# wbuntine/libstb

Measured on AMD Instinct MI355X. Metric: S-table cells/s, higher is better.
Workload: dtype f64

## Files before the change

include/stb_hip.h:

```cpp
#ifndef STB_HIP_H
#define STB_HIP_H

#include <stddef.h>
#include <stdint.h>

#ifdef __cplusplus
extern "C" {
#endif

const char *stb_last_error(void);
int stb_device_count(void);
int stb_device_name(char *buf, int len);

int stb_set_device(int dev);
int stb_get_device(void);
int stb_device_enter(int dev);
void stb_device_leave(int prev);

void *stb_device_malloc(size_t bytes);
void stb_device_free(void *p);
void *stb_host_malloc(size_t bytes);
void stb_host_free(void *p);
void *stb_host_malloc_huge(size_t bytes);
void stb_host_free_huge(void *p);
// ... 170 lines not shown
int stb_groups_aterms_multi(stb_groups_t *const *sets, int k, const double *x_host, int D, double *out_host);
int stb_groups_create_node(int ndev, int I, const int *K, const uint32_t *T, const uint32_t *nflat, const uint16_t *tflat,
                           const double *bpar, unsigned N, unsigned M, int Dmax, stb_groups_t **sets_out);
int stb_groups_aterms_device(stb_groups_t *g, const double *x_host, int D, double *d_out, void *stream);
int stb_groups_ssum_device(stb_groups_t *g, const double *x_host, int D, double *d_out, void *stream);
int stb_groups_ssum(stb_groups_t *g, const double *x_host, int D, double *out_host);
int stb_groups_aterms_tables(stb_groups_t *g, const double *x_host, int D, double *out_host);
double stb_groups_samplea(stb_groups_t *g, double a, void *rng, int loops, int verbose);
typedef struct stb_modea_info {
  int rounds, evals, at_bound;
  double lo, hi, g_lo, g_hi;
  double grad, delta;
} stb_modea_info_t;
int stb_groups_aterms_grad(stb_groups_t *g, const double *x_host, int D, double *val_out, double *grad_out);
int stb_groups_modea(stb_groups_t *g, double a_lo, double a_hi, double tol, int rounds_max, double *a_hat, double *curv,
                     stb_modea_info_t *info);
int stb_groups_update_restaurants(stb_groups_t *g, const uint32_t *T, const double *bpar);
int stb_groups_pairs_begin(stb_groups_t *g);
int stb_groups_pairs_put(stb_groups_t *g, const uint32_t *n, const uint16_t *t, uint64_t count, unsigned *maxn, unsigned *maxt);
int stb_groups_pairs_put_ragged(stb_groups_t *g, int I, const int *K, uint32_t *const *n, uint16_t *const *t, unsigned *maxn, unsigned *maxt);
int stb_groups_pairs_commit(stb_groups_t *g, const uint32_t *T, const double *bpar, unsigned N, unsigned M);
int stb_groups_update_pairs(stb_groups_t *g, const uint32_t *nflat, const uint16_t *tflat);
unsigned stb_groups_fallbacks(void);
int stb_grid_shape(unsigned N, unsigned M, int D, int *C_out, int *G_out, int *K_out);
int stb_groups_shape(const stb_groups_t *g, int *I, uint64_t *G, unsigned *N, unsigned *M, int *Dmax);
int stb_groups_last_form(const stb_groups_t *g, int *fused, int *which, int *sparse, int *C, int *R);
int stb_groups_aterms_timed(stb_groups_t *g, const double *x_host, int D, double *out_host,
                            float *ms_fill, float *ms_sweep, float *ms_terms);

int stb_sample_tcounts(const double *d_table, const double *d_S1, unsigned N, unsigned M, double a,
                       const double *d_bpar, int I, const uint64_t *d_koff , const uint32_t *d_n,
                       uint16_t *d_t, uint32_t *d_T, const double *d_h ,
                       uint64_t seed, uint64_t sweep, void *stream);
typedef struct stb_tcounts stb_tcounts_t;
stb_tcounts_t *stb_tcounts_create(int I, const int *K, const uint32_t *nflat, const uint16_t *tflat,
                                  const double *hflat, unsigned M );
int stb_tcounts_set_h(stb_tcounts_t *s, const double *hflat);
int stb_tcounts_sweep(stb_tcounts_t *s, double a, const double *bpar ,
                      uint64_t seed, uint64_t sweep, int nsweeps);
int stb_tcounts_get(stb_tcounts_t *s, uint16_t *t_out, uint32_t *T_out);
int stb_tcounts_to_groups(stb_tcounts_t *s, stb_groups_t *g, const double *bpar );
double stb_tcounts_sampleb(stb_tcounts_t *s, double b_in, double shape, double scale, double a, void *rng,
                           int loops, int verbose, uint64_t seed, uint64_t sweep);
void stb_tcounts_free(stb_tcounts_t *s);

#define STB_TC_REF_WINDOW 1u
// ... 213 lines not shown
```

libstb_amd/capi.py:

```python
from __future__ import annotations

import ctypes as C
import os
from functools import lru_cache

import numpy as np

_HERE = os.path.dirname(os.path.abspath(__file__))
LIB_PATH = os.environ.get("STB_LIB_PATH") or os.path.join(_HERE, "lib", "libstb_amd.so")

S_STABLE, S_UVTABLE, S_FLOAT, S_VERBOSE, S_QUITONBOUND, S_THREADS, S_ASYMPT = 1, 2, 4, 8, 16, 32, 64
FILL_SCALED, FILL_LOGDOMAIN, FILL_SCALED_STEP, FILL_SPLIT, FILL_FUSED, FILL_PC, FILL_CHAIN, FILL_CHAINX, FILL_CK, FILL_HB = 0, 1, 2, 3, 4, 5, 6, 7, 8, 9

c_double_p = C.POINTER(C.c_double)
c_u32_p = C.POINTER(C.c_uint32)
c_u16_p = C.POINTER(C.c_uint16)
c_int_p = C.POINTER(C.c_int)
c_float_p = C.POINTER(C.c_float)

LOGDENS = C.CFUNCTYPE(C.c_double, C.c_double, C.c_void_p)
GETVAL = C.CFUNCTYPE(None, c_u32_p, c_u16_p, C.c_uint, C.c_uint)


class StbError(RuntimeError):
# ... 98 lines not shown
    _fields_ = [("stages", C.c_int), ("accepted", C.c_int), ("evals", C.c_int), ("stage_pick", C.c_int),
                ("log_alpha", C.c_double), ("rect", C.c_double * 4), ("a_prop", C.c_double), ("b_prop", C.c_double),
                ("L_cur", C.c_double), ("L_prop", C.c_double), ("cell", C.c_int * 5), ("box", (C.c_int * 4) * 5),
                ("L", c_double_p)]


@lru_cache(maxsize=None)
def lib() -> C.CDLL:
    if not os.path.exists(LIB_PATH):
        raise StbError(
            f"{LIB_PATH} is missing: build it with `python -c 'import __graft_entry__ as g; g.build()'` "
            "or `make -C libstb_amd/csrc` (there is no pure-Python or CPU implementation)")
    try:
        import torch
    except Exception:
        pass
    L = C.CDLL(LIB_PATH)
    u, d, i, vp, u64, sz = C.c_uint, C.c_double, C.c_int, C.c_void_p, C.c_uint64, C.c_size_t

    ROUND5 = {"stb_groups_pairs_begin", "stb_groups_pairs_put", "stb_groups_pairs_put_ragged", "stb_groups_pairs_commit",
              "stb_groups_update_pairs", "stb_groups_fallbacks", "stb_grid_shape", "stb_bterms_update",
              "stb_table_probe", "stb_slow_launches", "stb_shared_gpu_mode", "stb_set_shared_gpu", "stb_note_launch_span",
              "stb_lookup_V", "stb_lookup_U", "stb_lookup_UV", "stb_groups_aterms_multi", "stb_groups_create_node",
              "stb_groups_last_form"}

    def sig(name, res, args):
        try:
            f = getattr(L, name)
        except AttributeError:
            if name in ROUND5 and os.environ.get("STB_LIB_PATH"):
                return
            raise
        f.restype = res
        f.argtypes = args

    sig("S_make", vp, [u, u, u, u, d, C.c_uint32])
    sig("S_tag", None, [vp, C.c_char_p])
    sig("S_remake", i, [vp, d])
    sig("S_free", None, [vp])
    for n in ("S_S", "S_U", "S_UV", "S_V", "S_asympt"):
        sig(n, d, [vp, u, u])
    sig("S_S1", d, [vp, u])
    sig("S_report", None, [vp, vp])
    sig("stb_extend_policy", None, [u, u, u, u, i, i, C.POINTER(u), C.POINTER(u)])
    sig("stb_table_sync", i, [vp])
    sig("stb_table_probe", None, [vp, i, C.POINTER(u), C.POINTER(u), sz, c_double_p])
    sig("stb_table_mirrored", None, [vp, C.POINTER(u), C.POINTER(u)])
# ... 46 lines not shown
    sig("stb_lookup_U", i, [vp, u, u, C.c_double, vp, vp, u64, vp, vp])
    sig("stb_lookup_UV", i, [vp, u, u, C.c_double, vp, vp, u64, vp, vp])
    sig("stb_sweep_workspace_bytes", sz, [u64, i])
    sig("stb_sweep_S", i, [vp, u64, vp, u64, i, u, u, vp, vp, u64, vp, vp, sz, vp])
    sig("stb_terms_workspace_bytes", sz, [u64, i])
    sig("stb_restaurant_terms", i, [c_double_p, i, vp, vp, u64, vp, vp, sz, vp])
    sig("stb_bterms", i, [c_double_p, i, d, d, d, vp, u64, vp, vp, sz, vp])
    sig("stb_groups_create", vp, [i, c_int_p, c_u32_p, c_u32_p, c_u16_p, c_double_p, u, u, i])
    sig("stb_groups_free", None, [vp])
    sig("stb_groups_aterms", i, [vp, c_double_p, i, c_double_p])
    sig("stb_groups_aterms_tables", i, [vp, c_double_p, i, c_double_p])
    sig("stb_groups_aterms_async", i, [vp, c_double_p, i, c_double_p, vp])
    sig("stb_groups_wait", i, [vp])
    sig("stb_groups_aterms_multi", i, [C.POINTER(vp), i, c_double_p, i, c_double_p])
    sig("stb_groups_create_node", i, [i, i, c_int_p, c_u32_p, c_u32_p, c_u16_p, c_double_p, u, u, i, C.POINTER(vp)])
    sig("stb_groups_aterms_device", i, [vp, c_double_p, i, vp, vp])
    sig("stb_groups_update_restaurants", i, [vp, c_u32_p, c_double_p])
    sig("stb_groups_pairs_begin", i, [vp])
    sig("stb_groups_pairs_put", i, [vp, c_u32_p, c_u16_p, u64, C.POINTER(u), C.POINTER(u)])
    sig("stb_groups_pairs_put_ragged", i, [vp, i, c_int_p, vp, vp, C.POINTER(u), C.POINTER(u)])
    sig("stb_groups_pairs_commit", i, [vp, c_u32_p, c_double_p, u, u])
    sig("stb_groups_update_pairs", i, [vp, c_u32_p, c_u16_p])
    sig("stb_groups_fallbacks", C.c_uint, [])
    sig("stb_grid_shape", i, [u, u, i, c_int_p, c_int_p, c_int_p])
    sig("stb_groups_shape", i, [vp, c_int_p, C.POINTER(u64), C.POINTER(u), C.POINTER(u), c_int_p])
    sig("stb_groups_last_form", i, [vp, c_int_p, c_int_p, c_int_p, c_int_p, c_int_p])
    sig("stb_sampler_cache_clear", None, [])
    sig("stb_groups_aterms_timed", i, [vp, c_double_p, i, c_double_p, c_float_p, c_float_p, c_float_p])
    sig("stb_sample_tcounts", i, [vp, vp, u, u, d, vp, i, vp, vp, vp, vp, vp, u64, u64, vp])
    sig("stb_tcounts_create", vp, [i, c_int_p, c_u32_p, c_u16_p, c_double_p, u])
    sig("stb_tcounts_set_h", i, [vp, c_double_p])
    sig("stb_tcounts_sweep", i, [vp, d, c_double_p, u64, u64, i])
    sig("stb_tcounts_get", i, [vp, c_u16_p, c_u32_p])
    sig("stb_tcounts_to_groups", i, [vp, vp, c_double_p])
    sig("stb_tcounts_free", None, [vp])
    sig("stb_sample_tcounts_window", i, [vp, vp, u, u, d, vp, i, vp, vp, vp, vp, vp, u, u, u64, u64, vp])
    sig("stb_tcounts_sweep_window", i, [vp, d, c_double_p, u, u, u64, u64, i])
    sig("stb_sample_tindic", i, [vp, u, u, d, vp, i, vp, vp, vp, vp, vp, vp, vp, u, u64, u64, vp])
    sig("stb_tindic_create", vp, [i, c_int_p, c_u32_p, c_u16_p, c_double_p, c_u32_p, u, u])
    sig("stb_tindic_set_h", i, [vp, c_double_p])
    sig("stb_tindic_sweep", i, [vp, d, c_double_p, u64, u64, i])
    sig("stb_tindic_get", i, [vp, c_u16_p, c_u32_p])
    sig("stb_tindic_to_groups", i, [vp, vp, c_double_p])
    sig("stb_tindic_free", None, [vp])
    sig("stb_sample_tdishes", i, [vp, u, u, d, vp, i, vp, vp, vp, vp, vp, vp, vp, vp, vp, u, u, u64, u64, vp, vp])
    sig("stb_tindic_set_classes", i, [vp, c_u32_p, u])
# ... 1189 lines not shown
```

libstb_amd/csrc/groups.h:

```cpp
#ifndef STB_GROUPS_H
#define STB_GROUPS_H

#include <vector>

#include "stb_common.h"

#define STB_TERMS_DMAX 64
#define STB_NLISTS 6
#define GH_JQ_HOST 64
#define STB_WS_FORM 4096

struct slab_info {
  int R, G, NQ, UC, HC;
  int PB;
  unsigned UCp;
  const unsigned *rec_off;
};

struct stb_cell_list {
  unsigned *item_ptr;
  unsigned short *ent_pos;
  unsigned *ent_cnt;
  unsigned *tile_off, *dense, *tinfo, *jobs, *tjob, *tnw, *toff;
  unsigned n_jobs;
  int ready, R, G;
  size_t ent_cap, dense_cap;
};
static inline bool stb_list_from_slab(const stb_cell_list &l) { return l.ent_cap != 0; }


struct stb_groups {
  int dev;
  int I;
  uint64_t G;
  unsigned N, M;
  int Dmax;
  uint32_t *d_n, *d_T;
  uint16_t *d_t;
  double *d_bpar;
  double *d_tables, *d_S1, *d_out;
// ... 28 lines not shown
  int pend_ssum;
  int sel_which;
  int last_fused, last_C, last_R;
  double *pend_out;
  double pend_x[STB_TERMS_DMAX];
  last_fill pend_fill;
  uint32_t *h_pn;
  uint16_t *h_pt;
  uint32_t *h_T;
  double *h_bpar;
  uint64_t put_n, flushed_n;
  unsigned put_maxn, put_maxt;
  int putting;
  int have_pairs;
  int have_bounds;
  int sorted;
  unsigned *d_slab;
  size_t slab_elems;
  int slab_which;
  int slab_R, slab_G, slab_UCp;
  unsigned slab_items;
  int slab_clean;
  unsigned *d_icnt;
  unsigned long long *d_ninf;
  void *d_scan_tmp;
  size_t scan_tmp_bytes;
  double *d_gtab, *d_dS1g, *d_gout;
  void *d_ws_da, *d_ws_dasweep;
  size_t ws_da, ws_dasweep;
  uint64_t da_stride, da_G;
  unsigned da_N, da_M;
};

static inline int stb_grid_which(int C) { return C == 2 ? 3 : (C == 4 ? 4 : 5); }
static inline int stb_which_C(int which) { return which == 3 ? 2 : (which == 4 ? 4 : 8); }
static inline int stb_pos_bits(int C) { return C == 8 ? 9 : 8; }

#if defined(__HIPCC__)
__device__ __forceinline__ unsigned stb_block_exclusive_1024(unsigned mine, unsigned *lds, unsigned *total) {
  const unsigned tid = threadIdx.x, lane = tid & 63, wave = tid >> 6;
  unsigned v = mine;
#pragma unroll
  for (int o = 1; o < 64; o <<= 1) {
    const unsigned u = __shfl_up(v, o, 64);
    if ((int)lane >= o) v += u;
  }
  if (lane == 63) lds[wave] = v;
  __syncthreads();
  if (tid == 0) {
// ... 7 lines not shown
  }
  __syncthreads();
  const unsigned ex = lds[wave] + v - mine;
  if (total) *total = lds[16];
  __syncthreads();
  return ex;
}
#endif

#define STB_DENSE_NWMAX 40
#define STB_DENSE_CSR 63u

void stb_grid_tile_offsets(const grid_geom &g, std::vector<unsigned> &off);

void stb_list_release(stb_cell_list &l, bool with_shape);
void stb_lists_drop(stb_groups_t *g, bool keep_capacity);
void stb_list_request(const stb_groups_t *g, int which, dot_request *req);
int stb_lists_build(stb_groups_t *g, int which, int D);
int stb_lists_slab_build(stb_groups_t *g, int which, int D, const hb_dot_info &H, const grid_geom &gg);
int stb_lists_jobs_device(stb_groups_t *g, int which, int D, const grid_geom &gg, const unsigned *tnw);
int stb_lists_jobs_from(stb_groups_t *g, int which, int D, const grid_geom &gg, const unsigned *h_nw);
int stb_lists_sort_build(stb_groups_t *g, int which, int D, const hb_dot_info &H, const grid_geom &gg);
void stb_groups_new_pairs(stb_groups_t *g, int reused);
int stb_groups_set_bounds(stb_groups_t *g, unsigned N, unsigned M);
int stb_groups_sort_pairs(stb_groups_t *g);
int stb_groups_alloc_dotp(stb_groups_t *g);

struct stb_counts_view {
  int dev, I;
  uint64_t G;
  unsigned maxn, Mdraw;
  const uint32_t *d_n, *d_T;
  const uint16_t *d_t;
  const double *d_bpar;
  bool resident;
  hipStream_t st;
  const char *noun;
};
int stb_groups_take_counts(stb_groups_t *g, const stb_counts_view &v, const double *bpar, const char *who);

#endif
```

libstb_amd/csrc/groups.hip:

```cpp

#include <rocprim/device/device_radix_sort.hpp>

#include <atomic>

#include "groups.h"

__global__ void k_pack_pairs(const uint32_t *n, const uint16_t *t, uint64_t G, uint64_t *key) {
  uint64_t g = (uint64_t)blockIdx.x * blockDim.x + threadIdx.x;
  if (g < G) key[g] = ((uint64_t)n[g] << 16) | t[g];
}
__global__ void k_unpack_pairs(const uint64_t *key, uint64_t G, uint32_t *n, uint16_t *t) {
  uint64_t g = (uint64_t)blockIdx.x * blockDim.x + threadIdx.x;
  if (g < G) {
    n[g] = (uint32_t)(key[g] >> 16);
    t[g] = (uint16_t)(key[g] & 0xffff);
  }
}

static int sort_pairs(uint32_t *d_n, uint16_t *d_t, uint64_t G, hipStream_t st) {
  if (G < 2) return 0;
  uint64_t *k0 = nullptr, *k1 = nullptr;
  void *tmp = nullptr;
  size_t tmp_bytes = 0;
  int rc = 1;
// ... 15 lines not shown
    if (rocprim::radix_sort_keys(tmp, tmp_bytes, k0, k1, (size_t)G, 0, 48, st) != hipSuccess) {
      stb_fail("sort_pairs: radix_sort_keys failed");
      break;
    }
    hipLaunchKernelGGL(k_unpack_pairs, dim3(blocks), dim3(256), 0, st, k1, G, d_n, d_t);
    if (hipStreamSynchronize(st) != hipSuccess) {
      stb_fail("sort_pairs: %s", hipGetErrorString(hipGetLastError()));
      break;
    }
    rc = 0;
  } while (0);
  if (rc != 0) (void)hipStreamSynchronize(st);
  stb_pool_free(k0);
  stb_pool_free(k1);
  stb_pool_free(tmp);
  return rc;
}

extern "C" void stb_groups_free(stb_groups_t *g) {
  STB_ENTRY;
  if (!g) return;
  stb_device_scope dev(g->dev);
  std::vector<void *> ptrs = {g->d_n, g->d_T, g->d_t, g->d_bpar, g->d_tables, g->d_S1, g->d_out, g->d_ws_fill, g->d_ws_sweep, g->d_ws_terms,
                              g->d_cnt, g->d_n2, g->d_t2, g->d_dotp, g->d_slab, g->d_icnt, g->d_ninf, g->d_scan_tmp,
                              g->d_gtab, g->d_dS1g, g->d_gout, g->d_ws_da, g->d_ws_dasweep};
  if (g->st) (void)hipStreamSynchronize(g->st);
  for (void *p : ptrs) stb_pool_free(p);
  for (stb_cell_list &l : g->lists) stb_list_release(l, true);
  stb_pool_free(g->h_out);
  stb_pool_free(g->h_pn);
  stb_pool_free(g->h_pt);
  stb_pool_free(g->h_T);
  stb_pool_free(g->h_bpar);
  if (g->ev_dep) (void)hipEventDestroy(g->ev_dep);
  if (g->ev_done) (void)hipEventDestroy(g->ev_done);
  for (auto &e : g->ev)
    if (e) (void)hipEventDestroy(e);
  if (g->st) (void)hipStreamDestroy(g->st);
  free(g);
}

#define GCHK(expr)                                                                            \
  do {                                                                                        \
    hipError_t e_ = (expr);                                                                   \
    if (e_ != hipSuccess) {                                                                   \
      stb_fail("%s failed: %s (%s:%d)", #expr, hipGetErrorString(e_), __FILE__, __LINE__);        \
      stb_groups_free(g);                                                                     \
// ... 709 lines not shown
```

libstb_amd/csrc/lists.hip:

```cpp
#include <rocprim/device/device_scan.hpp>

#include <algorithm>

#include "groups.h"


__device__ __forceinline__ int slab_word(unsigned nn, unsigned tt, unsigned N, unsigned M, const slab_info &H, unsigned &item, size_t &idx) {
  if (nn <= 1 || nn == tt) return 0;
  if (tt == 0 || nn < tt || tt > M || nn > N) return 1;
  unsigned j = 0, col = 0;
  if (tt >= 2) {
    const unsigned e = tt - 2;
    j = e / (unsigned)H.UC;
    col = 1 + (e - j * (unsigned)H.UC);
  }
  const unsigned b = (nn - 2) / (unsigned)H.R, r = (nn - 2) - b * (unsigned)H.R;
  const unsigned b0 = (j * (unsigned)H.UC) / (unsigned)H.R;
  const unsigned rec = H.rec_off[j + 1] + (b - b0);
  const unsigned q = r / (unsigned)H.G;
  item = rec * (unsigned)H.NQ + q;
  idx = ((size_t)item * (unsigned)H.G + (r - q * (unsigned)H.G)) * H.UCp + col;
  return 2;
}

__global__ __launch_bounds__(256) void k_count_cells(const uint32_t *n, const uint16_t *t, uint64_t G, unsigned N, unsigned M, slab_info H,
                                                     unsigned *slab, unsigned long long *ninf) {
  const uint64_t g = (uint64_t)blockIdx.x * blockDim.x + threadIdx.x;
  int kind = 0;
  unsigned item = 0;
  size_t idx = 0;
  if (g < G) kind = slab_word(n[g], t[g], N, M, H, item, idx);
  if (kind == 2) __hip_atomic_fetch_add(&slab[idx], 1u, __ATOMIC_RELAXED, __HIP_MEMORY_SCOPE_AGENT);
  const unsigned long long m = __ballot(kind == 1);
  if (m && (threadIdx.x & 63) == 0) atomicAdd(ninf, (unsigned long long)__popcll(m));
}

__global__ __launch_bounds__(256) void k_item_count(const unsigned *slab, unsigned nitems, unsigned len, unsigned *icnt) {
  const unsigned item = blockIdx.x * 4 + (threadIdx.x >> 6), lane = threadIdx.x & 63;
  if (item >= nitems) return;
  const unsigned *w = slab + (size_t)item * len;
  unsigned c = 0;
  unsigned k = lane * 4;
  if ((((size_t)item * len) & 3u) == 0) {
    for (; k + 3 < len; k += 256) {
      const uint4 v = *reinterpret_cast<const uint4 *>(w + k);
      c += (v.x != 0u) + (v.y != 0u) + (v.z != 0u) + (v.w != 0u);
    }
    for (unsigned i = (len & ~3u) + lane; i < len; i += 64) c += w[i] != 0u;
  } else {
    for (unsigned i = lane; i < len; i += 64) c += w[i] != 0u;
  }
#pragma unroll
  for (int o = 32; o >= 1; o >>= 1) c += __shfl_xor(c, o);
  if (lane == 0) icnt[item] = c;
}

__global__ __launch_bounds__(256) void k_emit_cells(unsigned *slab, const unsigned *item_ptr, unsigned nitems, slab_info H, unsigned short *ent_pos,
// ... 172 lines not shown
  if (!with_shape) return;
  void **shaped[] = {(void **)&l.tile_off, (void **)&l.tnw, (void **)&l.toff};
  for (void **p : shaped) free_z(*p);
  l.n_jobs = 0;
  l.ready = 0;
}

void stb_lists_drop(stb_groups_t *g, bool keep_capacity) {
  for (stb_cell_list &l : g->lists) {
    if (!keep_capacity || !stb_list_from_slab(l)) stb_list_release(l, true);
    l.ready = 0;
    l.n_jobs = 0;
  }
  FREE_Z(g->d_n2);
  FREE_Z(g->d_t2);
  FREE_Z(g->d_cnt);
  g->G2 = 0;
  g->n_inf = 0;
  g->fused_ready = 0;
  g->sparse = 0;
  if (!keep_capacity) {
    FREE_Z(g->d_slab);
    FREE_Z(g->d_icnt);
    FREE_Z(g->d_scan_tmp);
    FREE_Z(g->d_dotp);
    g->slab_elems = 0;
    g->slab_which = 0;
    g->scan_tmp_bytes = 0;
    g->dotp_elems = 0;
  }
}

void stb_list_request(const stb_groups_t *g, int which, dot_request *req) {
  const stb_cell_list &l = g->lists[which];
  req->item_ptr = l.item_ptr;
  req->ent_pos = l.ent_pos;
  req->ent_cnt = l.ent_cnt;
  req->nsg = g->nsg;
  req->col0 = which >= 3 ? 4 : which + 1;
  if (which == 2) req->geom_C = g->hb_sum_C;
  if (which >= 3) {
    req->geom_C = stb_which_C(which);
    req->geom_R = l.R;
    req->geom_G = l.G;
    req->tile_off = l.tile_off;
    req->dense = l.dense;
    req->tinfo = l.tinfo;
    req->jobs = l.jobs;
    req->tjob = l.tjob;
  }
}

static size_t slab_limit_bytes() { return (size_t)stb_env_int("STB_SLAB_MB", 4096) << 20; }

int stb_lists_slab_build(stb_groups_t *g, int which, int D, const hb_dot_info &H, const grid_geom &gg) {
  if (which < 2 || !stb_env_int("STB_LISTS_SLAB", 1)) return 2;
  stb_cell_list &l = g->lists[which];
  const unsigned N = g->N, M = g->M;
  const uint64_t G = g->G;
  if (G == 0 || G >= 0xffffffffull) return 2;
  if (G * 3 > stb_table_cells(N, M)) return 2;
  slab_info S;
  S.R = H.R;
  S.G = H.G;
  S.NQ = H.NQ;
  S.UC = H.UC;
  S.HC = H.HC;
  S.UCp = (unsigned)H.UC + 1u;
  S.rec_off = H.rec_off;
  const uint64_t nitems64 = (uint64_t)H.n_rec * (unsigned)H.NQ;
  const uint64_t elems64 = nitems64 * (unsigned)H.G * S.UCp;
  if (nitems64 >= (1ull << 31) || elems64 * 4 > slab_limit_bytes()) return 2;
  S.PB = which >= 3 ? stb_pos_bits(H.C) : 8;
  if (H.G > 32 || H.HC - 1 + (int)S.UCp > (1 << S.PB)) return 2;
  if (which >= 3 && (size_t)H.NQ * ((size_t)(g->G / 64) + H.n_tiles + 1) >= (1u << 26)) return 2;
  const unsigned nitems = (unsigned)nitems64;
  const size_t elems = (size_t)elems64;
  hipStream_t st = g->st;
  if (!g->d_slab || g->slab_elems < elems || g->slab_which != which || g->slab_R != H.R || g->slab_G != H.G || g->slab_UCp != (int)S.UCp ||
      g->slab_items != nitems) {
    if (g->d_slab) HIPCHK(hipStreamSynchronize(st));
    if (!g->d_slab || g->slab_elems < elems) {
      FREE_Z(g->d_slab);
      g->slab_elems = 0;
      if (stb_pool_malloc((void **)&g->d_slab, 4 * elems) != hipSuccess) return stb_fail("stb_groups_aterms: out of device memory (count slab, %zu MB)", (4 * elems) >> 20);
      g->slab_elems = elems;
      g->slab_clean = 0;
    }
    FREE_Z(g->d_icnt);
    if (stb_pool_malloc((void **)&g->d_icnt, 4 * ((size_t)nitems + 2)) != hipSuccess || (!g->d_ninf && stb_pool_malloc((void **)&g->d_ninf, 64) != hipSuccess))
      return stb_fail("stb_groups_aterms: out of device memory");
    HIPCHK(hipMemsetAsync(g->d_icnt, 0, 4 * ((size_t)nitems + 2), st));
    size_t need = 0;
    if (rocprim::exclusive_scan(nullptr, need, g->d_icnt, g->d_icnt, 0u, (size_t)nitems + 1, rocprim::plus<unsigned>(), st) != hipSuccess)
      return stb_fail("stb_groups_aterms: exclusive_scan (size query) failed");
    if (which >= 3) {
      size_t need2 = 0;
      if (rocprim::exclusive_scan(nullptr, need2, g->d_icnt, g->d_icnt, 0u, (size_t)H.n_tiles + 1, rocprim::plus<unsigned>(), st) != hipSuccess)
        return stb_fail("stb_groups_aterms: exclusive_scan (size query) failed");
      if (need2 > need) need = need2;
    }
    if (need > g->scan_tmp_bytes) {
      FREE_Z(g->d_scan_tmp);
      if (stb_pool_malloc(&g->d_scan_tmp, need ? need : 1) != hipSuccess) return stb_fail("stb_groups_aterms: out of device memory");
      g->scan_tmp_bytes = need ? need : 1;
    }
    g->slab_which = which;
    g->slab_R = H.R;
    g->slab_G = H.G;
    g->slab_UCp = (int)S.UCp;
    g->slab_items = nitems;
  }
  if (!g->slab_clean) HIPCHK(hipMemsetAsync(g->d_slab, 0, 4 * g->slab_elems, st));
  if (l.ent_cap < G || !l.item_ptr) {
    if (l.ent_pos) HIPCHK(hipStreamSynchronize(st));
    FREE_Z(l.ent_pos);
    FREE_Z(l.ent_cnt);
    FREE_Z(l.item_ptr);
    if (stb_pool_malloc((void **)&l.ent_pos, 2 * (size_t)G + 256) != hipSuccess || stb_pool_malloc((void **)&l.ent_cnt, 4 * (size_t)G + 256) != hipSuccess ||
        stb_pool_malloc((void **)&l.item_ptr, 4 * ((size_t)nitems + 2)) != hipSuccess)
      return stb_fail("stb_groups_aterms: out of device memory");
    l.ent_cap = (size_t)G;
  }
  g->slab_clean = 0;
  HIPCHK(hipMemsetAsync(g->d_ninf, 0, 8, st));
  hipLaunchKernelGGL(k_count_cells, dim3((unsigned)((G + 255) / 256)), dim3(256), 0, st, g->d_n, g->d_t, G, N, M, S, g->d_slab, g->d_ninf);
  hipLaunchKernelGGL(k_item_count, dim3((nitems + 3) / 4), dim3(256), 0, st, g->d_slab, nitems, (unsigned)H.G * S.UCp, g->d_icnt);
  if (which < 3) {
    size_t tb = g->scan_tmp_bytes;
    if (rocprim::exclusive_scan(g->d_scan_tmp, tb, g->d_icnt, l.item_ptr, 0u, (size_t)nitems + 1, rocprim::plus<unsigned>(), st) != hipSuccess)
      return stb_fail("stb_groups_aterms: exclusive_scan failed");
    hipLaunchKernelGGL(k_emit_cells, dim3((nitems + 3) / 4), dim3(256), 0, st, g->d_slab, l.item_ptr, nitems, S, l.ent_pos,
                       l.ent_cnt);
    HIPCHK(hipGetLastError());
    g->slab_clean = 1;
  } else {
    const unsigned n_tiles = H.n_tiles, NQ = (unsigned)H.NQ;
    const size_t words_cap = (size_t)NQ * ((size_t)(G / 64) + n_tiles + 1);
    if (words_cap >= (1u << 26)) return stb_fail("stb_groups_aterms: a dense list beyond 2^32 bytes");
    {
      unsigned **bufs[] = {&l.tnw, &l.toff, &l.tinfo};
      for (unsigned **q : bufs)
        if (!*q && stb_pool_malloc((void **)q, 4 * (size_t)(n_tiles + 2)) != hipSuccess) return stb_fail("stb_groups_aterms: out of device memory");
    }
    if (l.dense_cap < words_cap || !l.dense) {
      if (l.dense) HIPCHK(hipStreamSynchronize(st));
      FREE_Z(l.dense);
      if (stb_pool_malloc((void **)&l.dense, 256 * words_cap) != hipSuccess) return stb_fail("stb_groups_aterms: out of device memory");
      l.dense_cap = words_cap;
    }
    hipLaunchKernelGGL(k_scan_lists, dim3(1), dim3(1024), 0, st, g->d_icnt, nitems, n_tiles, NQ, l.item_ptr, l.tnw, l.toff,
                       l.tinfo);
    hipLaunchKernelGGL(k_emit_both, dim3((nitems + 3) / 4), dim3(256), 0, st, g->d_slab, l.item_ptr, nitems, S, l.ent_pos,
                       l.ent_cnt, NQ, S.PB + 5, l.tnw, l.toff, l.tinfo, l.dense);
    HIPCHK(hipGetLastError());
    g->slab_clean = 1;
    if (stb_lists_jobs_device(g, which, D, gg, l.tnw)) return 1;
  }
  if (!g->d_dotp && stb_groups_alloc_dotp(g)) return 1;
  g->sparse = 1;
  l.ready = 1;
  l.R = H.R;
  l.G = H.G;
  g->fused_ready = 1;
  g->nsg = (M + 63) / 64 + 4;
  return 0;
}

static unsigned jobs_rule(const grid_geom &gg, int D, int *jlim) {
  unsigned nwh = (unsigned)stb_env_int("STB_GRID_HELP_NW", 0);
  if (nwh < 1) {
    const double waves_per_simd = (double)gg.JW * D / (4.0 * stb_cu_count());
    nwh = waves_per_simd <= 1.9 ? 4 : (waves_per_simd <= 2.7 ? 6 : 8);
  }
  *jlim = ((gg.JW - 1) / gg.P) * gg.P;
  if (*jlim > 64) *jlim = 64;
  return nwh;
}
static int jobs_room(stb_cell_list &l, unsigned n_tiles) {
  if (!l.jobs && stb_pool_malloc((void **)&l.jobs, 4 * ((size_t)n_tiles + 128 + 1)) != hipSuccess) return stb_fail("stb_groups_aterms: out of device memory");
  if (!l.tjob && stb_pool_malloc((void **)&l.tjob, 4 * (size_t)(n_tiles + 1)) != hipSuccess) return stb_fail("stb_groups_aterms: out of device memory");
  return 0;
}

__global__ __launch_bounds__(1024) void k_jobs_build(const unsigned *tnw, unsigned n_tiles, const unsigned *tile_off, int JW, int jlim, int R, int UC, int NB,
                                                     unsigned cap, unsigned nwh0, unsigned *jobs, unsigned *tjob) {
  __shared__ unsigned hist[64], s_nwh, s_scan[17], s_off[1024];
  const unsigned tid = threadIdx.x;
// ... 126 lines not shown
static int resolve_layout(const stb_groups_t *g, int &which, int D, hb_dot_info &H, grid_geom &gg) {
  memset(&H, 0, sizeof(H));
  memset(&gg, 0, sizeof(gg));
  if (which == 2 && stb_hb_dot_info(g->N, g->M, g->Dmax, &H, g->hb_sum_C)) return stb_fail("stb_groups_aterms: no halo-block geometry for N=%u M=%u", g->N, g->M);
  if (which < 3) return 0;
  if (stb_grid_geometry(g->N, g->M, D, &gg)) return stb_fail("stb_groups_aterms: no grid geometry for N=%u M=%u", g->N, g->M);
  which = stb_grid_which(gg.C);
  H.R = gg.R;
  H.UC = gg.U * gg.C;
  H.HC = gg.HL * gg.C;
  H.NB = gg.NB;
  H.JW = gg.JW;
  H.NQ = gg.NQ;
  H.G = gg.G;
  H.C = gg.C;
  H.n_tiles = H.n_rec = gg.n_tiles;
  return 0;
}

static int match_strip_shape(stb_groups_t *g, stb_cell_list &l, hb_dot_info &H, const grid_geom &gg) {
  if ((l.ready || l.tile_off) && (l.R != H.R || l.G != H.G)) {
    (void)hipStreamSynchronize(g->st);
    stb_list_release(l, true);
  }
  if (!l.ready && !l.tile_off) {
    std::vector<unsigned> off;
    stb_grid_tile_offsets(gg, off);
    if (stb_pool_malloc((void **)&l.tile_off, off.size() * sizeof(unsigned)) != hipSuccess ||
        hipMemcpy(l.tile_off, off.data(), off.size() * sizeof(unsigned), hipMemcpyHostToDevice) != hipSuccess)
      return stb_fail("stb_groups_aterms: out of device memory");
  }
  H.rec_off = l.tile_off;
  return 0;
}

int stb_lists_build(stb_groups_t *g, int which, int D) {
  hb_dot_info H;
  grid_geom gg;
  if (resolve_layout(g, which, D, H, gg)) return 1;
  stb_cell_list &l = g->lists[which];
  if (which >= 3 && match_strip_shape(g, l, H, gg)) return 1;
  if (l.ready) return 0;
  const int rc = stb_lists_slab_build(g, which, D, H, gg);
  return rc != 2 ? rc : stb_lists_sort_build(g, which, D, H, gg);
}
```

libstb_amd/csrc/pairs.hip:

```cpp
#include <algorithm>
#include <vector>

#include <pthread.h>
#include <sched.h>

#include "groups.h"

void stb_groups_new_pairs(stb_groups_t *g, int reused) {
  stb_lists_drop(g, true);
  g->sorted = 0;
  g->have_pairs = 1;
  g->reused = reused;
}



#define STB_PUT_CHUNK (256u * 1024u)

extern "C" int stb_groups_pairs_begin(stb_groups_t *g) {
  STB_ENTRY;
  if (!g) return stb_fail("stb_groups_pairs_begin: null group set");
  if (g->pending == 1) return stb_fail("stb_groups_pairs_begin: an evaluation queued with stb_groups_aterms_async has not been waited for");
  stb_device_scope dev(g->dev);
  g->put_n = g->flushed_n = 0;
  g->put_maxn = g->put_maxt = 0;
  g->putting = 0;
  if (hipStreamSynchronize(g->st) != hipSuccess) return stb_fail("stb_groups_pairs_begin: %s", hipGetErrorString(hipGetLastError()));
  if (g->G && ((!g->h_pn && stb_pool_malloc((void **)&g->h_pn, 4 * (size_t)g->G, 1) != hipSuccess) ||
               (!g->h_pt && stb_pool_malloc((void **)&g->h_pt, 2 * (size_t)g->G, 1) != hipSuccess)))
    return stb_fail("stb_groups_pairs_begin: out of pinned host memory");
  g->putting = 1;
  return 0;
}

static unsigned copy_max_u32(uint32_t *__restrict d, const uint32_t *__restrict s, size_t n, unsigned m) {
  for (size_t i = 0; i < n; i++) {
    const uint32_t v = s[i];
    d[i] = v;
    m = v > m ? v : m;
  }
  return m;
}
static unsigned copy_max_u16(uint16_t *__restrict d, const uint16_t *__restrict s, size_t n, unsigned m) {
  uint16_t mm = 0;
  for (size_t i = 0; i < n; i++) {
    const uint16_t v = s[i];
    d[i] = v;
    mm = v > mm ? v : mm;
  }
  return mm > m ? mm : m;
}

static int put_flush(stb_groups_t *g, bool all) {
  while (g->put_n - g->flushed_n >= (all ? 1u : STB_PUT_CHUNK)) {
    const uint64_t c = all ? g->put_n - g->flushed_n : STB_PUT_CHUNK;
    const uint64_t o = g->flushed_n;
    HIPCHK(hipMemcpyAsync(g->d_n + o, g->h_pn + o, 4 * c, hipMemcpyHostToDevice, g->st));
    HIPCHK(hipMemcpyAsync(g->d_t + o, g->h_pt + o, 2 * c, hipMemcpyHostToDevice, g->st));
    g->flushed_n += c;
  }
  return 0;
}

extern "C" int stb_groups_pairs_put(stb_groups_t *g, const uint32_t *n, const uint16_t *t, uint64_t count, unsigned *maxn, unsigned *maxt) {
  if (!g || !g->putting) return stb_fail("stb_groups_pairs_put: stb_groups_pairs_begin comes first");
  if (g->put_n + count > g->G) return stb_fail("stb_groups_pairs_put: %llu pairs for a set of %llu", (unsigned long long)(g->put_n + count), (unsigned long long)g->G);
  if (count) {
    g->put_maxn = copy_max_u32(g->h_pn + g->put_n, n, count, g->put_maxn);
    g->put_maxt = copy_max_u16(g->h_pt + g->put_n, t, count, g->put_maxt);
    g->put_n += count;
  }
  if (maxn) *maxn = g->put_maxn;
  if (maxt) *maxt = g->put_maxt;
  if (g->put_n - g->flushed_n < STB_PUT_CHUNK) return 0;
  stb_device_scope dev(g->dev);
  return put_flush(g, false);
}

extern "C" int stb_groups_pairs_commit(stb_groups_t *g, const uint32_t *T, const double *bpar, unsigned N, unsigned M) {
  STB_ENTRY;
  if (!g || !g->putting) return stb_fail("stb_groups_pairs_commit: stb_groups_pairs_begin comes first");
  if (g->put_n != g->G) return stb_fail("stb_groups_pairs_commit: %llu of the set's %llu pairs supplied", (unsigned long long)g->put_n, (unsigned long long)g->G);
  stb_device_scope dev(g->dev);
  g->putting = 0;
  if (put_flush(g, true)) return 1;
  if (N == 0 || M == 0) {
    if (!g->have_bounds) return stb_fail("stb_groups_pairs_commit: the set has no table bounds yet");
    N = g->N;
    M = g->M;
  }
  if (stb_groups_set_bounds(g, N, M)) return 1;
  stb_groups_new_pairs(g, 0);
  if (T && bpar && g->I > 0) {
    memcpy(g->h_T, T, sizeof(uint32_t) * (size_t)g->I);
    memcpy(g->h_bpar, bpar, sizeof(double) * (size_t)g->I);
    if (hipMemcpyAsync(g->d_T, g->h_T, sizeof(uint32_t) * (size_t)g->I, hipMemcpyHostToDevice, g->st) != hipSuccess ||
        hipMemcpyAsync(g->d_bpar, g->h_bpar, sizeof(double) * (size_t)g->I, hipMemcpyHostToDevice, g->st) != hipSuccess)
      return stb_fail("stb_groups_pairs_commit: %s", hipGetErrorString(hipGetLastError()));
  }
  return 0;
}

#include <atomic>
#include <condition_variable>
#include <memory>
#include <mutex>
#include <thread>

namespace {
struct put_slice {
  int i0, i1;
  uint64_t off, count;
  std::atomic<uint64_t> done;
  unsigned maxn, maxt;
};
// ... 162 lines not shown
      if (!use_lk.owns_lock()) P = nullptr;
    }
  }
  if (P) {
    {
      std::lock_guard<std::mutex> lk(P->mu);
      P->job = &J;
      P->gen++;
    }
    P->cv.notify_all();
  }
  int rc = 0;
  {
    stb_device_scope dev(g->dev);
    if (!P) put_run(&J);
    uint64_t flushed = 0;
    int k = 0;
    while (k < J.nslices && !rc) {
      put_slice &S = slices[(size_t)k];
      const uint64_t d = S.done.load(std::memory_order_acquire);
      const uint64_t upto = S.off + d;
      if (d == S.count) k++;
      if (upto - flushed >= 131072 || (k == J.nslices && upto > flushed)) {
        if (hipMemcpyAsync(g->d_n + flushed, g->h_pn + flushed, 4 * (upto - flushed), hipMemcpyHostToDevice, g->st) != hipSuccess ||
            hipMemcpyAsync(g->d_t + flushed, g->h_pt + flushed, 2 * (upto - flushed), hipMemcpyHostToDevice, g->st) != hipSuccess)
          rc = stb_fail("stb_groups_pairs_put_ragged: %s", hipGetErrorString(hipGetLastError()));
        flushed = upto;
      } else if (d != S.count) {
        if (!put_step(&J)) __builtin_ia32_pause();
      }
    }
  }
  if (P) {
    std::unique_lock<std::mutex> lk(P->mu);
    P->job = nullptr;
    P->cv.wait(lk, [&] { return P->busy == 0; });
  }
  if (rc) return rc;
  unsigned mn = 0, mt = 0;
  for (int k = 0; k < ns; k++) {
    mn = slices[(size_t)k].maxn > mn ? slices[(size_t)k].maxn : mn;
    mt = slices[(size_t)k].maxt > mt ? slices[(size_t)k].maxt : mt;
  }
  g->put_n = g->flushed_n = G;
  g->put_maxn = mn;
  g->put_maxt = mt;
  if (maxn) *maxn = mn;
  if (maxt) *maxt = mt;
  return 0;
// ... 15 lines not shown
```

Measured before the change: 218.8 billion.

## Fuse pair upload with slab cell counting via zero-copy take kernel

Replaces the host-to-device memcpy of pair chunks with a kernel that reads pinned host memory directly, writes the pairs to device buffers, and, when the previous slab layout is known to still match, counts slab cells and per-item occupancy during the upload. Per-item counts go into replicated counters that are folded afterwards, so the later list build can skip the separate count and item-count kernels and the slab memset. This overlaps counting with the transfer but adds zero-copy PCIe reads, an extra memset of the replicas, and complex validity bookkeeping that could produce wrong lists if the layout check misses a case.

```diff
diff --git a/include/stb_hip.h b/include/stb_hip.h
--- a/include/stb_hip.h
+++ b/include/stb_hip.h
@@ -216,6 +216,7 @@
 int stb_groups_pairs_commit(stb_groups_t *g, const uint32_t *T, const double *bpar, unsigned N, unsigned M);
 int stb_groups_update_pairs(stb_groups_t *g, const uint32_t *nflat, const uint16_t *tflat);
 unsigned stb_groups_fallbacks(void);
+unsigned stb_groups_takes(void);
 int stb_grid_shape(unsigned N, unsigned M, int D, int *C_out, int *G_out, int *K_out);
 int stb_groups_shape(const stb_groups_t *g, int *I, uint64_t *G, unsigned *N, unsigned *M, int *Dmax);
 int stb_groups_last_form(const stb_groups_t *g, int *fused, int *which, int *sparse, int *C, int *R);
diff --git a/libstb_amd/capi.py b/libstb_amd/capi.py
--- a/libstb_amd/capi.py
+++ b/libstb_amd/capi.py
@@ -144,7 +144,8 @@
               "stb_groups_update_pairs", "stb_groups_fallbacks", "stb_grid_shape", "stb_bterms_update",
               "stb_table_probe", "stb_slow_launches", "stb_shared_gpu_mode", "stb_set_shared_gpu", "stb_note_launch_span",
               "stb_lookup_V", "stb_lookup_U", "stb_lookup_UV", "stb_groups_aterms_multi", "stb_groups_create_node",
-              "stb_groups_last_form"}
+              "stb_groups_last_form",
+              "stb_groups_takes"}
 
     def sig(name, res, args):
         try:
@@ -237,6 +238,7 @@
     sig("stb_groups_pairs_commit", i, [vp, c_u32_p, c_double_p, u, u])
     sig("stb_groups_update_pairs", i, [vp, c_u32_p, c_u16_p])
     sig("stb_groups_fallbacks", C.c_uint, [])
+    sig("stb_groups_takes", C.c_uint, [])
     sig("stb_grid_shape", i, [u, u, i, c_int_p, c_int_p, c_int_p])
     sig("stb_groups_shape", i, [vp, c_int_p, C.POINTER(u64), C.POINTER(u), C.POINTER(u), c_int_p])
     sig("stb_groups_last_form", i, [vp, c_int_p, c_int_p, c_int_p, c_int_p, c_int_p])
diff --git a/libstb_amd/csrc/groups.h b/libstb_amd/csrc/groups.h
--- a/libstb_amd/csrc/groups.h
+++ b/libstb_amd/csrc/groups.h
@@ -7,6 +7,7 @@
 
 #define STB_TERMS_DMAX 64
 #define STB_NLISTS 6
+#define STB_ICNT_REPS 32
 #define GH_JQ_HOST 64
 #define STB_WS_FORM 4096
 
@@ -16,6 +17,15 @@
   unsigned UCp;
   const unsigned *rec_off;
 };
+struct slab_mark {
+  int which;
+  unsigned N, M, items;
+  slab_info S;
+};
+static inline bool stb_slab_mark_same(const slab_mark &a, const slab_mark &b) {
+  return a.which == b.which && a.N == b.N && a.M == b.M && a.items == b.items && a.S.R == b.S.R && a.S.G == b.S.G && a.S.NQ == b.S.NQ && a.S.UC == b.S.UC &&
+         a.S.HC == b.S.HC && a.S.PB == b.S.PB && a.S.UCp == b.S.UCp && a.S.rec_off == b.S.rec_off;
+}
 
 struct stb_cell_list {
   unsigned *item_ptr;
@@ -90,9 +100,21 @@
   unsigned slab_items;
   int slab_clean;
   unsigned *d_icnt;
+  unsigned *d_irep;
+  unsigned irep_stride;
   unsigned long long *d_ninf;
   void *d_scan_tmp;
   size_t scan_tmp_bytes;
+  uint32_t *h_pn_dev;
+  uint16_t *h_pt_dev;
+  int take_on;
+  int built_valid;
+  int built_matched;
+  int built_D;
+  slab_mark built_for;
+  int armed;
+  slab_mark armed_for;
+  int counted;
   double *d_gtab, *d_dS1g, *d_gout;
   void *d_ws_da, *d_ws_dasweep;
   size_t ws_da, ws_dasweep;
@@ -146,6 +168,8 @@
 int stb_lists_jobs_from(stb_groups_t *g, int which, int D, const grid_geom &gg, const unsigned *h_nw);
 int stb_lists_sort_build(stb_groups_t *g, int which, int D, const hb_dot_info &H, const grid_geom &gg);
 void stb_groups_new_pairs(stb_groups_t *g, int reused);
+int stb_lists_arm(stb_groups_t *g);
+int stb_take_pairs(stb_groups_t *g, uint64_t o, uint64_t c);
 int stb_groups_set_bounds(stb_groups_t *g, unsigned N, unsigned M);
 int stb_groups_sort_pairs(stb_groups_t *g);
 int stb_groups_alloc_dotp(stb_groups_t *g);
diff --git a/libstb_amd/csrc/groups.hip b/libstb_amd/csrc/groups.hip
--- a/libstb_amd/csrc/groups.hip
+++ b/libstb_amd/csrc/groups.hip
@@ -61,7 +61,7 @@
   if (!g) return;
   stb_device_scope dev(g->dev);
   std::vector<void *> ptrs = {g->d_n, g->d_T, g->d_t, g->d_bpar, g->d_tables, g->d_S1, g->d_out, g->d_ws_fill, g->d_ws_sweep, g->d_ws_terms,
-                              g->d_cnt, g->d_n2, g->d_t2, g->d_dotp, g->d_slab, g->d_icnt, g->d_ninf, g->d_scan_tmp,
+                              g->d_cnt, g->d_n2, g->d_t2, g->d_dotp, g->d_slab, g->d_icnt, g->d_irep, g->d_ninf, g->d_scan_tmp,
                               g->d_gtab, g->d_dS1g, g->d_gout, g->d_ws_da, g->d_ws_dasweep};
   if (g->st) (void)hipStreamSynchronize(g->st);
   for (void *p : ptrs) stb_pool_free(p);
diff --git a/libstb_amd/csrc/lists.hip b/libstb_amd/csrc/lists.hip
--- a/libstb_amd/csrc/lists.hip
+++ b/libstb_amd/csrc/lists.hip
@@ -1,8 +1,12 @@
 #include <rocprim/device/device_scan.hpp>
 
 #include <algorithm>
+#include <atomic>
 
 #include "groups.h"
+
+static std::atomic<unsigned> g_list_takes{0};
+extern "C" unsigned stb_groups_takes(void) { return g_list_takes.load(); }
 
 
 __device__ __forceinline__ int slab_word(unsigned nn, unsigned tt, unsigned N, unsigned M, const slab_info &H, unsigned &item, size_t &idx) {
@@ -33,6 +37,62 @@
   if (kind == 2) __hip_atomic_fetch_add(&slab[idx], 1u, __ATOMIC_RELAXED, __HIP_MEMORY_SCOPE_AGENT);
   const unsigned long long m = __ballot(kind == 1);
   if (m && (threadIdx.x & 63) == 0) atomicAdd(ninf, (unsigned long long)__popcll(m));
+}
+
+__global__ __launch_bounds__(256) void k_take_pairs(const uint32_t *__restrict hn, const uint16_t *__restrict ht, uint32_t *__restrict dn, uint16_t *__restrict dt,
+                                                    uint64_t o, uint64_t c, int count, unsigned N, unsigned M, slab_info H, unsigned *slab, unsigned *irep,
+                                                    unsigned stride, unsigned long long *ninf) {
+  const uint64_t g0 = (o / 4 + (uint64_t)blockIdx.x * blockDim.x + threadIdx.x) * 4, end = o + c;
+  unsigned nn[4] = {0u, 0u, 0u, 0u}, tt[4] = {0u, 0u, 0u, 0u};
+  bool in[4];
+#pragma unroll
+  for (int j = 0; j < 4; j++) in[j] = g0 + j >= o && g0 + j < end;
+  if (in[0] && in[3]) {
+    const uint4 a = *reinterpret_cast<const uint4 *>(hn + g0);
+    const uint2 b = *reinterpret_cast<const uint2 *>(ht + g0);
+    *reinterpret_cast<uint4 *>(dn + g0) = a;
+    *reinterpret_cast<uint2 *>(dt + g0) = b;
+    nn[0] = a.x, nn[1] = a.y, nn[2] = a.z, nn[3] = a.w;
+    tt[0] = b.x & 0xffffu, tt[1] = b.x >> 16, tt[2] = b.y & 0xffffu, tt[3] = b.y >> 16;
+  } else {
+#pragma unroll
+    for (int j = 0; j < 4; j++)
+      if (in[j]) {
+        nn[j] = hn[g0 + j];
+        tt[j] = ht[g0 + j];
+        dn[g0 + j] = nn[j];
+        dt[g0 + j] = (uint16_t)tt[j];
+      }
+  }
+  if (!count) return;
+  int kind[4];
+  unsigned item[4], old[4] = {1u, 1u, 1u, 1u}, inf = 0;
+  size_t idx[4];
+#pragma unroll
+  for (int j = 0; j < 4; j++) {
+    kind[j] = 0;
+    item[j] = 0;
+    idx[j] = 0;
+    if (in[j]) kind[j] = slab_word(nn[j], tt[j], N, M, H, item[j], idx[j]);
+  }
+#pragma unroll
+  for (int j = 0; j < 4; j++)
+    if (kind[j] == 2) old[j] = __hip_atomic_fetch_add(&slab[idx[j]], 1u, __ATOMIC_RELAXED, __HIP_MEMORY_SCOPE_AGENT);
+#pragma unroll
+  for (int j = 0; j < 4; j++) {
+    if (old[j] == 0u) __hip_atomic_fetch_add(&irep[(size_t)(threadIdx.x & (STB_ICNT_REPS - 1)) * stride + item[j]], 1u, __ATOMIC_RELAXED, __HIP_MEMORY_SCOPE_AGENT);
+    inf += (unsigned)__popcll(__ballot(kind[j] == 1));
+  }
+  if (inf && (threadIdx.x & 63) == 0) atomicAdd(ninf, (unsigned long long)inf);
+}
+
+__global__ __launch_bounds__(256) void k_item_fold(const unsigned *irep, unsigned stride, unsigned nitems, unsigned *icnt) {
+  const unsigned item = blockIdx.x * 256 + threadIdx.x;
+  if (item >= nitems) return;
+  unsigned c = 0;
+#pragma unroll 8
+  for (int r = 0; r < STB_ICNT_REPS; r++) c += irep[(size_t)r * stride + item];
+  icnt[item] = c;
 }
 
 __global__ __launch_bounds__(256) void k_item_count(const unsigned *slab, unsigned nitems, unsigned len, unsigned *icnt) {
@@ -251,10 +311,12 @@
   if (!keep_capacity) {
     FREE_Z(g->d_slab);
     FREE_Z(g->d_icnt);
+    FREE_Z(g->d_irep);
     FREE_Z(g->d_scan_tmp);
     FREE_Z(g->d_dotp);
     g->slab_elems = 0;
     g->slab_which = 0;
+    g->built_valid = g->counted = g->armed = 0;
     g->scan_tmp_bytes = 0;
     g->dotp_elems = 0;
   }
@@ -282,14 +344,13 @@
 
 static size_t slab_limit_bytes() { return (size_t)stb_env_int("STB_SLAB_MB", 4096) << 20; }
 
-int stb_lists_slab_build(stb_groups_t *g, int which, int D, const hb_dot_info &H, const grid_geom &gg) {
+static int slab_geometry(const stb_groups_t *g, int which, const hb_dot_info &H, slab_mark &mk, size_t &elems) {
   if (which < 2 || !stb_env_int("STB_LISTS_SLAB", 1)) return 2;
-  stb_cell_list &l = g->lists[which];
   const unsigned N = g->N, M = g->M;
   const uint64_t G = g->G;
   if (G == 0 || G >= 0xffffffffull) return 2;
   if (G * 3 > stb_table_cells(N, M)) return 2;
-  slab_info S;
+  slab_info &S = mk.S;
   S.R = H.R;
   S.G = H.G;
   S.NQ = H.NQ;
@@ -303,11 +364,31 @@
   S.PB = which >= 3 ? stb_pos_bits(H.C) : 8;
   if (H.G > 32 || H.HC - 1 + (int)S.UCp > (1 << S.PB)) return 2;
   if (which >= 3 && (size_t)H.NQ * ((size_t)(g->G / 64) + H.n_tiles + 1) >= (1u << 26)) return 2;
-  const unsigned nitems = (unsigned)nitems64;
-  const size_t elems = (size_t)elems64;
+  mk.which = which;
+  mk.N = N;
+  mk.M = M;
+  mk.items = (unsigned)nitems64;
+  elems = (size_t)elems64;
+  return 0;
+}
+static bool slab_laid_for(const stb_groups_t *g, const slab_mark &mk, size_t elems) {
+  return g->d_slab && g->slab_elems >= elems && g->slab_which == mk.which && g->slab_R == mk.S.R && g->slab_G == mk.S.G && g->slab_UCp == (int)mk.S.UCp &&
+         g->slab_items == mk.items;
+}
+
+int stb_lists_slab_build(stb_groups_t *g, int which, int D, const hb_dot_info &H, const grid_geom &gg) {
+  slab_mark mk;
+  size_t elems = 0;
+  if (slab_geometry(g, which, H, mk, elems)) return 2;
+  stb_cell_list &l = g->lists[which];
+  const unsigned N = g->N, M = g->M;
+  const uint64_t G = g->G;
+  const slab_info S = mk.S;
+  const unsigned nitems = mk.items;
+  const bool taken = g->counted && stb_slab_mark_same(g->armed_for, mk) && slab_laid_for(g, mk, elems) && g->d_icnt && g->d_irep && g->d_ninf;
+  g->counted = 0;
   hipStream_t st = g->st;
-  if (!g->d_slab || g->slab_elems < elems || g->slab_which != which || g->slab_R != H.R || g->slab_G != H.G || g->slab_UCp != (int)S.UCp ||
-      g->slab_items != nitems) {
+  if (!slab_laid_for(g, mk, elems)) {
     if (g->d_slab) HIPCHK(hipStreamSynchronize(st));
     if (!g->d_slab || g->slab_elems < elems) {
       FREE_Z(g->d_slab);
@@ -317,7 +398,10 @@
       g->slab_clean = 0;
     }
     FREE_Z(g->d_icnt);
-    if (stb_pool_malloc((void **)&g->d_icnt, 4 * ((size_t)nitems + 2)) != hipSuccess || (!g->d_ninf && stb_pool_malloc((void **)&g->d_ninf, 64) != hipSuccess))
+    FREE_Z(g->d_irep);
+    g->irep_stride = (nitems + 2u + 31u) & ~31u;
+    if (stb_pool_malloc((void **)&g->d_icnt, 4 * ((size_t)nitems + 2)) != hipSuccess ||
+        stb_pool_malloc((void **)&g->d_irep, 4 * (size_t)STB_ICNT_REPS * g->irep_stride) != hipSuccess || (!g->d_ninf && stb_pool_malloc((void **)&g->d_ninf, 64) != hipSuccess))
       return stb_fail("stb_groups_aterms: out of device memory");
     HIPCHK(hipMemsetAsync(g->d_icnt, 0, 4 * ((size_t)nitems + 2), st));
     size_t need = 0;
@@ -340,7 +424,7 @@
     g->slab_UCp = (int)S.UCp;
     g->slab_items = nitems;
   }
-  if (!g->slab_clean) HIPCHK(hipMemsetAsync(g->d_slab, 0, 4 * g->slab_elems, st));
+  if (!taken && !g->slab_clean) HIPCHK(hipMemsetAsync(g->d_slab, 0, 4 * g->slab_elems, st));
   if (l.ent_cap < G || !l.item_ptr) {
     if (l.ent_pos) HIPCHK(hipStreamSynchronize(st));
     FREE_Z(l.ent_pos);
@@ -352,9 +436,14 @@
     l.ent_cap = (size_t)G;
   }
   g->slab_clean = 0;
-  HIPCHK(hipMemsetAsync(g->d_ninf, 0, 8, st));
-  hipLaunchKernelGGL(k_count_cells, dim3((unsigned)((G + 255) / 256)), dim3(256), 0, st, g->d_n, g->d_t, G, N, M, S, g->d_slab, g->d_ninf);
-  hipLaunchKernelGGL(k_item_count, dim3((nitems + 3) / 4), dim3(256), 0, st, g->d_slab, nitems, (unsigned)H.G * S.UCp, g->d_icnt);
+  if (taken) {
+    g_list_takes.fetch_add(1);
+    hipLaunchKernelGGL(k_item_fold, dim3((nitems + 255) / 256), dim3(256), 0, st, g->d_irep, g->irep_stride, nitems, g->d_icnt);
+  } else {
+    HIPCHK(hipMemsetAsync(g->d_ninf, 0, 8, st));
+    hipLaunchKernelGGL(k_count_cells, dim3((unsigned)((G + 255) / 256)), dim3(256), 0, st, g->d_n, g->d_t, G, N, M, S, g->d_slab, g->d_ninf);
+    hipLaunchKernelGGL(k_item_count, dim3((nitems + 3) / 4), dim3(256), 0, st, g->d_slab, nitems, (unsigned)H.G * S.UCp, g->d_icnt);
+  }
   if (which < 3) {
     size_t tb = g->scan_tmp_bytes;
     if (rocprim::exclusive_scan(g->d_scan_tmp, tb, g->d_icnt, l.item_ptr, 0u, (size_t)nitems + 1, rocprim::plus<unsigned>(), st) != hipSuccess)
@@ -393,6 +482,53 @@
   l.G = H.G;
   g->fused_ready = 1;
   g->nsg = (M + 63) / 64 + 4;
+  g->built_matched = !g->built_valid || stb_slab_mark_same(g->built_for, mk);
+  g->built_valid = 1;
+  g->built_for = mk;
+  g->built_D = D;
+  return 0;
+}
+
+static int resolve_layout(const stb_groups_t *g, int &which, int D, hb_dot_info &H, grid_geom &gg);
+
+int stb_lists_arm(stb_groups_t *g) {
+  g->armed = 0;
+  g->counted = 0;
+  if (!g->take_on || !g->built_valid || !g->built_matched || !g->slab_clean || !g->have_bounds || !g->d_slab || !g->d_icnt || !g->d_irep || !g->d_ninf) return 0;
+  int which = g->built_for.which;
+  hb_dot_info H;
+  grid_geom gg;
+  if (resolve_layout(g, which, g->built_D, H, gg)) return 0;
+  if (which >= 3) {
+    const stb_cell_list &l = g->lists[which];
+    if (!l.tile_off || l.R != H.R || l.G != H.G) return 0;
+    H.rec_off = l.tile_off;
+  }
+  slab_mark mk;
+  size_t elems = 0;
+  if (slab_geometry(g, which, H, mk, elems) || !stb_slab_mark_same(mk, g->built_for) || !slab_laid_for(g, mk, elems)) return 0;
+  if (g->irep_stride < mk.items) return 0;
+  HIPCHK(hipMemsetAsync(g->d_irep, 0, 4 * (size_t)STB_ICNT_REPS * g->irep_stride, g->st));
+  HIPCHK(hipMemsetAsync(g->d_ninf, 0, 8, g->st));
+  g->armed_for = mk;
+  g->armed = 1;
+  return 0;
+}
+
+int stb_take_pairs(stb_groups_t *g, uint64_t o, uint64_t c) {
+  if (!c) return 0;
+  if (o + c > g->G || !g->h_pn_dev || !g->h_pt_dev) return stb_fail("stb_groups_pairs: pairs %llu + %llu of %llu", (unsigned long long)o, (unsigned long long)c, (unsigned long long)g->G);
+  const uint64_t quads = (o + c + 3) / 4 - o / 4;
+  if (quads + 255 >= (1ull << 39)) return stb_fail("stb_groups_pairs: a piece of %llu pairs", (unsigned long long)c);
+  slab_info S;
+  memset(&S, 0, sizeof(S));
+  if (g->armed) {
+    S = g->armed_for.S;
+    g->slab_clean = 0;
+  }
+  hipLaunchKernelGGL(k_take_pairs, dim3((unsigned)((quads + 255) / 256)), dim3(256), 0, g->st, g->h_pn_dev, g->h_pt_dev, g->d_n, g->d_t, o, c, g->armed, g->N, g->M, S,
+                     g->d_slab, g->d_irep, g->irep_stride, g->d_ninf);
+  HIPCHK(hipGetLastError());
   return 0;
 }
 
@@ -565,6 +701,7 @@
   if ((l.ready || l.tile_off) && (l.R != H.R || l.G != H.G)) {
     (void)hipStreamSynchronize(g->st);
     stb_list_release(l, true);
+    g->built_valid = g->counted = 0;
   }
   if (!l.ready && !l.tile_off) {
     std::vector<unsigned> off;
@@ -585,5 +722,7 @@
   if (which >= 3 && match_strip_shape(g, l, H, gg)) return 1;
   if (l.ready) return 0;
   const int rc = stb_lists_slab_build(g, which, D, H, gg);
-  return rc != 2 ? rc : stb_lists_sort_build(g, which, D, H, gg);
-}
+  if (rc != 2) return rc;
+  g->built_valid = g->counted = 0;
+  return stb_lists_sort_build(g, which, D, H, gg);
+}
diff --git a/libstb_amd/csrc/pairs.hip b/libstb_amd/csrc/pairs.hip
--- a/libstb_amd/csrc/pairs.hip
+++ b/libstb_amd/csrc/pairs.hip
@@ -8,6 +8,7 @@
 
 void stb_groups_new_pairs(stb_groups_t *g, int reused) {
   stb_lists_drop(g, true);
+  g->counted = 0;
   g->sorted = 0;
   g->have_pairs = 1;
   g->reused = reused;
@@ -29,6 +30,11 @@
   if (g->G && ((!g->h_pn && stb_pool_malloc((void **)&g->h_pn, 4 * (size_t)g->G, 1) != hipSuccess) ||
                (!g->h_pt && stb_pool_malloc((void **)&g->h_pt, 2 * (size_t)g->G, 1) != hipSuccess)))
     return stb_fail("stb_groups_pairs_begin: out of pinned host memory");
+  g->take_on = stb_env_int("STB_PAIRS_TAKE", 1) != 0;
+  if (g->take_on && g->h_pn && g->h_pt && (!g->h_pn_dev || !g->h_pt_dev) &&
+      (hipHostGetDevicePointer((void **)&g->h_pn_dev, g->h_pn, 0) != hipSuccess || hipHostGetDevicePointer((void **)&g->h_pt_dev, g->h_pt, 0) != hipSuccess))
+    return stb_fail("stb_groups_pairs_begin: %s", hipGetErrorString(hipGetLastError()));
+  if (stb_lists_arm(g)) return 1;
   g->putting = 1;
   return 0;
 }
@@ -51,12 +57,18 @@
   return mm > m ? mm : m;
 }
 
+static int put_piece(stb_groups_t *g, uint64_t o, uint64_t c) {
+  if (g->take_on) return stb_take_pairs(g, o, c);
+  HIPCHK(hipMemcpyAsync(g->d_n + o, g->h_pn + o, 4 * c, hipMemcpyHostToDevice, g->st));
+  HIPCHK(hipMemcpyAsync(g->d_t + o, g->h_pt + o, 2 * c, hipMemcpyHostToDevice, g->st));
+  return 0;
+}
+
 static int put_flush(stb_groups_t *g, bool all) {
   while (g->put_n - g->flushed_n >= (all ? 1u : STB_PUT_CHUNK)) {
     const uint64_t c = all ? g->put_n - g->flushed_n : STB_PUT_CHUNK;
     const uint64_t o = g->flushed_n;
-    HIPCHK(hipMemcpyAsync(g->d_n + o, g->h_pn + o, 4 * c, hipMemcpyHostToDevice, g->st));
-    HIPCHK(hipMemcpyAsync(g->d_t + o, g->h_pt + o, 2 * c, hipMemcpyHostToDevice, g->st));
+    if (put_piece(g, o, c)) return 1;
     g->flushed_n += c;
   }
   return 0;
@@ -91,6 +103,10 @@
   }
   if (stb_groups_set_bounds(g, N, M)) return 1;
   stb_groups_new_pairs(g, 0);
+  if (g->armed) {
+    g->counted = 1;
+    g->armed = 0;
+  }
   if (T && bpar && g->I > 0) {
     memcpy(g->h_T, T, sizeof(uint32_t) * (size_t)g->I);
     memcpy(g->h_bpar, bpar, sizeof(double) * (size_t)g->I);
@@ -299,9 +315,7 @@
       const uint64_t upto = S.off + d;
       if (d == S.count) k++;
       if (upto - flushed >= 131072 || (k == J.nslices && upto > flushed)) {
-        if (hipMemcpyAsync(g->d_n + flushed, g->h_pn + flushed, 4 * (upto - flushed), hipMemcpyHostToDevice, g->st) != hipSuccess ||
-            hipMemcpyAsync(g->d_t + flushed, g->h_pt + flushed, 2 * (upto - flushed), hipMemcpyHostToDevice, g->st) != hipSuccess)
-          rc = stb_fail("stb_groups_pairs_put_ragged: %s", hipGetErrorString(hipGetLastError()));
+        rc = put_piece(g, flushed, upto - flushed);
         flushed = upto;
       } else if (d != S.count) {
         if (!put_step(&J)) __builtin_ia32_pause();
```

New measurement: 218.2 billion. About the same (-0.3%).
